# DefaultRui/VLN-VER

Measured on AMD Instinct MI355X. Metric: viewpoints/sec (multi-view->voxel fwd+bwd), vocc.py config, higher is better.
Workload: dtype bf16

## Files before the change

vln-ver_amd/csrc/ver_wgrad.hip:

```cpp
#include <cstdlib>
#include "ver_common.h"

namespace {
typedef __bf16 bf16x8 __attribute__((ext_vector_type(8)));
typedef float f32x16 __attribute__((ext_vector_type(16)));
typedef short s16x4 __attribute__((ext_vector_type(4)));
typedef short s16x8 __attribute__((ext_vector_type(8)));
typedef __attribute__((address_space(3))) s16x4 lds_s16x4;
typedef __attribute__((address_space(3))) void lds_void;

constexpr int kTile = 256;
constexpr int kSlabRows = 16;
constexpr int kSlabBytes = 2 * kSlabRows * kTile * 2;
constexpr int kRing = 8;
constexpr int kLdsBytes = kRing * kSlabBytes;

typedef int i32x2 __attribute__((ext_vector_type(2)));
typedef int i32x4 __attribute__((ext_vector_type(4)));

template <int OFF>
__device__ __forceinline__ i32x2 tr_read(int addr) {
    i32x2 v;
    asm volatile("ds_read_b64_tr_b16 %0, %1 offset:%2" : "=v"(v) : "v"(addr), "n"(OFF) : "memory");
    return v;
}
__device__ __forceinline__ bf16x8 frag(i32x2 lo, i32x2 hi) {
    return __builtin_bit_cast(bf16x8, (i32x4)__builtin_shufflevector(lo, hi, 0, 1, 2, 3));
}

struct WgradArgs {
    const __bf16* A;
    const __bf16* G;
    float* ws;
    long lda, ldg, M, Mc;
    int S, Ka, N, tiles_n, T;
    void* out;
    long ldo;
    int out_bf16;
    const __bf16* lattice;
    long lattice_bytes;
    const __bf16* cst;
    long cst_bytes;
    int B, H, W, C, P, CW, ncst, nseg;
    int seg_start[65];
    signed char kind[64], dz[64], dy[64], dx[64];
};

constexpr int kOutsideW = (int)0x80000000;
template <int L>
__device__ __forceinline__ int wcell_off(const WgradArgs& t, int b, int zl, int y, int x, int dz) {
    if ((unsigned)y >= (unsigned)t.H || (unsigned)x >= (unsigned)t.W) return kOutsideW;
    const int j = dz >> 1;
    int v;
    if (L == 0)
        v = ((b * 4 + zl + dz) * t.H + y) * t.W + x;
    else if (L == 2)
        v = ((((b * 2 + zl) * t.H + y) * t.W + x) << 1) + j;
    else
        v = (((((((y & 1) << 1 | (x & 1)) * t.B + b) * 2 + zl) * (t.H >> 1) + (y >> 1)) * (t.W >> 1) + (x >> 1)) << 1) + j;
    return v * t.C * 2;
}

struct WTapLane {
    int taddr;
    int boff;
    int bstep;
    int pend;
    int tend;
    int rows_left;
    int vo;
};

template <int L>
__device__ __forceinline__ int wtap_table_entry(const WgradArgs& t, int seg, int pos) {
    if (seg < 0) return kOutsideW;
    if (t.kind[seg]) return (pos * t.ncst + t.dz[seg]) * t.CW * 2;
    const int hw = t.H * t.W;
    const int zl = pos / hw, rem = pos - zl * hw;
    const int y = rem / t.W, x = rem - y * t.W;
    return wcell_off<L>(t, 0, zl, y + t.dy[seg], x + t.dx[seg], t.dz[seg]);
}

__device__ __forceinline__ int lds_read_b32(int addr) {
    int v;
    asm volatile("ds_read_b32 %0, %1" : "=v"(v) : "v"(addr) : "memory");
    return v;
}

__device__ __forceinline__ void wtap_step(const WgradArgs& t, WTapLane& tl, int tfetched) {
    tl.boff += tl.pend;
    tl.rows_left -= kSlabRows;
    tl.vo = tl.rows_left > 0 ? (int)((unsigned)tfetched + (unsigned)tl.boff) : kOutsideW;
    tl.taddr += 4 * kSlabRows;
    tl.pend = 0;
    if (tl.taddr >= tl.tend) tl.taddr -= 4 * t.P, tl.pend = tl.bstep;
}

struct WgradLane {
    int offA0, offA1, offB0, offB1;
    int voA, voG;
    int stepA, stepG;
    int dmaoff;
};

template <int SLOT>
__device__ __forceinline__ void read_slab(const WgradLane& c, i32x2 (&al)[4], i32x2 (&ah)[4], i32x2 (&bl)[2], i32x2 (&bh)[2]) {
    constexpr int SB = (SLOT & 3) * kSlabBytes;
    constexpr int UP = SLOT >= 4 ? 65536 : 0;
    const int a0 = c.offA0 + UP, a1 = c.offA1 + UP, b0 = c.offB0 + UP, b1 = c.offB1 + UP;
    al[0] = tr_read<SB>(a0);
    ah[0] = tr_read<SB + 512>(a0);
    bl[0] = tr_read<SB>(b0);
    bh[0] = tr_read<SB + 512>(b0);
    al[1] = tr_read<SB>(a1);
    ah[1] = tr_read<SB + 512>(a1);
    bl[1] = tr_read<SB>(b1);
    bh[1] = tr_read<SB + 512>(b1);
    al[2] = tr_read<SB + 1024>(a0);
    ah[2] = tr_read<SB + 1536>(a0);
    al[3] = tr_read<SB + 1024>(a1);
    ah[3] = tr_read<SB + 1536>(a1);
}

template <int PS, int KP, int PF, int IMPL>
__device__ __forceinline__ void phase(char* lds, f32x16 (&acc)[4][2], const WgradLane& c, __amdgpu_buffer_rsrc_t ra,
                                      __amdgpu_buffer_rsrc_t rg, unsigned& soA, unsigned& soG, const WgradArgs& t, WTapLane& tl) {
    i32x2 al[KP][4], ah[KP][4], bl[KP][2], bh[KP][2];
    int tnext = 0;
    read_slab<PS * KP>(c, al[0], ah[0], bl[0], bh[0]);
    if constexpr (KP == 2) read_slab<PS * KP + 1>(c, al[KP - 1], ah[KP - 1], bl[KP - 1], bh[KP - 1]);
#pragma unroll
    for (int u = 0; u < KP; ++u) {
        const int ds = (PS * KP + u + PF) % kRing;
        if constexpr (IMPL < 0) {
            __builtin_amdgcn_raw_ptr_buffer_load_lds(ra, (lds_void*)(lds + ds * kSlabBytes + c.dmaoff), 16, c.voA, (int)soA, 0, 0);
        } else {
            static_assert(IMPL < 0 || KP == 1, "implicit A: one slab per phase");
            __builtin_amdgcn_raw_ptr_buffer_load_lds(ra, (lds_void*)(lds + ds * kSlabBytes + c.dmaoff), 16, tl.vo, 0, 0, 0);
            tnext = lds_read_b32(tl.taddr);
        }
        __builtin_amdgcn_raw_ptr_buffer_load_lds(rg, (lds_void*)(lds + ds * kSlabBytes + kSlabBytes / 2 + c.dmaoff), 16, c.voG, (int)soG, 0, 0);
        soA += (unsigned)c.stepA;
        soG += (unsigned)c.stepG;
    }
    asm volatile("s_waitcnt vmcnt(%0)" ::"n"(2 * (PF - KP)) : "memory");
    __builtin_amdgcn_s_barrier();
    asm volatile("s_waitcnt lgkmcnt(0)"
                 : "+v"(al[0][0]), "+v"(ah[0][0]), "+v"(al[0][1]), "+v"(ah[0][1]), "+v"(al[0][2]), "+v"(ah[0][2]), "+v"(al[0][3]),
                   "+v"(ah[0][3]), "+v"(bl[0][0]), "+v"(bh[0][0]), "+v"(bl[0][1]), "+v"(bh[0][1]), "+v"(tnext)
                 :
                 : "memory");

    if constexpr (KP == 2)
        asm volatile(""
                     : "+v"(al[KP - 1][0]), "+v"(ah[KP - 1][0]), "+v"(al[KP - 1][1]), "+v"(ah[KP - 1][1]), "+v"(al[KP - 1][2]),
                       "+v"(ah[KP - 1][2]), "+v"(al[KP - 1][3]), "+v"(ah[KP - 1][3]), "+v"(bl[KP - 1][0]), "+v"(bh[KP - 1][0]),
                       "+v"(bl[KP - 1][1]), "+v"(bh[KP - 1][1])
                     :
                     : "memory");
    bf16x8 a[KP][4], b[KP][2];
#pragma unroll
    for (int u = 0; u < KP; ++u) {
#pragma unroll
        for (int i = 0; i < 4; ++i) a[u][i] = frag(al[u][i], ah[u][i]);
        b[u][0] = frag(bl[u][0], bh[u][0]);
        b[u][1] = frag(bl[u][1], bh[u][1]);
    }
    __builtin_amdgcn_sched_barrier(0);
    __builtin_amdgcn_s_setprio(1);
#pragma unroll
    for (int u = 0; u < KP; ++u)
#pragma unroll
        for (int it = 0; it < 4; ++it)
#pragma unroll
            for (int jt = 0; jt < 2; ++jt)
                acc[it][jt] = __builtin_amdgcn_mfma_f32_32x32x16_bf16(a[u][it], b[u][jt], acc[it][jt], 0, 0, 0);
    __builtin_amdgcn_s_setprio(0);
    __builtin_amdgcn_sched_barrier(0);
    if constexpr (IMPL >= 0) {
        wtap_step(t, tl, tnext);
        __builtin_amdgcn_sched_barrier(0);
    }
    __builtin_amdgcn_s_barrier();
}

template <int PS, int KP, int PF, int IMPL>
__device__ __forceinline__ void phases_from(int left, char* lds, f32x16 (&acc)[4][2], const WgradLane& c,
                                            __amdgpu_buffer_rsrc_t ra, __amdgpu_buffer_rsrc_t rg, unsigned& soA, unsigned& soG,
                                            const WgradArgs& t, WTapLane& tl) {
    if constexpr (PS < kRing / KP) {
        if (left > PS * KP) {
            phase<PS, KP, PF, IMPL>(lds, acc, c, ra, rg, soA, soG, t, tl);
            phases_from<PS + 1, KP, PF, IMPL>(left, lds, acc, c, ra, rg, soA, soG, t, tl);
        }
    }
}

template <int KP, int PF, int IMPL>
__device__ __forceinline__ void wgrad_body(const WgradArgs& p) {
    static_assert(PF >= KP && PF + (KP == 1 ? 2 : 4) <= kRing, "prefetch distance against the ring (WAR on the slot)");
    extern __shared__ __attribute__((aligned(1024))) char lds[];
    const int tid = threadIdx.x, lane = tid & 63;
    const int wave = __builtin_amdgcn_readfirstlane(tid >> 6);
    const int wr = wave >> 2, wc = wave & 3;
    int chunk, tile;
    {
        const int b = blockIdx.x;
        if ((p.S & 7) == 0) {
            const int xcd = b & 7, idx = b >> 3;
            chunk = xcd + 8 * (idx / p.T);
            tile = idx % p.T;
        } else {
            chunk = b / p.T;
            tile = b % p.T;
        }
    }
    const int mt = tile / p.tiles_n, nt = tile - mt * p.tiles_n;
    const long row0 = (long)chunk * p.Mc;
    const long rows = max(0L, min(p.Mc, p.M - row0));
    const int nslab = (int)((rows + kSlabRows * KP - 1) / (kSlabRows * KP)) * KP;

    const __bf16* ab = IMPL < 0 ? p.A + row0 * p.lda + (long)mt * kTile : nullptr;
    const __bf16* gb = p.G + row0 * p.ldg + (long)nt * kTile;
    const long abytes = ((p.M - row0 - 1) * p.lda + p.Ka - (long)mt * kTile) * 2;
    const long gbytes = ((p.M - row0 - 1) * p.ldg + p.N - (long)nt * kTile) * 2;
    const __amdgpu_buffer_rsrc_t rg = __builtin_amdgcn_make_buffer_rsrc((void*)gb, 0, (int)max(0L, min(gbytes, 0xFFFFFFFFL)), 0x00020000);
    WgradLane c;
    const int prow = lane >> 3, pch = (lane & 7) ^ (((prow >> 1) & 1) << 2);
    WTapLane tl = {};
    bool a_cst = false;
    if constexpr (IMPL >= 0) {
        int* tables = reinterpret_cast<int*>(lds + kLdsBytes);
        auto seg_of = [&](int col0) {
            int seg = -1;
            for (int i = 0; i < p.nseg; ++i)
                if (col0 >= p.seg_start[i] && col0 < p.seg_start[i + 1]) seg = i;
            return seg;
        };
        for (int q = 0; q < 4; ++q) {
            const int seg = seg_of(mt * kTile + 64 * q);
            for (int i = tid; i < p.P; i += 512) tables[q * p.P + i] = wtap_table_entry<IMPL>(p, seg, i);
        }
        __syncthreads();
        const int col0 = mt * kTile + 64 * (wave & 3);
        const int seg = seg_of(col0);
        a_cst = seg >= 0 && p.kind[seg];
        const long r = row0 + 8 * (wave >> 2) + prow;
        const int b0 = (int)(r / p.P), pos0 = (int)(r - (long)b0 * p.P);
        tl.bstep = a_cst ? 0 : (IMPL == 3 ? p.H * p.W : 4 * p.H * p.W) * p.C * 2;
        tl.boff = b0 * tl.bstep + (seg < 0 ? 0 : (col0 - p.seg_start[seg]) * 2) + pch * 16;
        const int lbase = (int)(uintptr_t)(__attribute__((address_space(3))) char*)(lds + kLdsBytes) + (wave & 3) * p.P * 4;
        tl.tend = lbase + 4 * p.P;
        tl.taddr = lbase + 4 * pos0;
        tl.pend = 0;
        tl.rows_left = (int)min(min(p.M, row0 + p.Mc) - r, 0x7FFFFFF0L) + kSlabRows;
        int t0 = lds_read_b32(tl.taddr);
        asm volatile("s_waitcnt lgkmcnt(0)" : "+v"(t0)::"memory");
        wtap_step(p, tl, t0);
    }
    const __amdgpu_buffer_rsrc_t ra =
        IMPL < 0 ? __builtin_amdgcn_make_buffer_rsrc((void*)ab, 0, (int)max(0L, min(abytes, 0xFFFFFFFFL)), 0x00020000)
                 : __builtin_amdgcn_make_buffer_rsrc((void*)(a_cst ? p.cst : p.lattice), 0,
                                                     (int)max(0L, min(a_cst ? p.cst_bytes : p.lattice_bytes, 0x7FFFFFFFL)), 0x00020000);
    c.voA = (int)(((8 * (wave >> 2) + prow) * p.lda + 64 * (wave & 3)) * 2) + pch * 16;
    c.voG = (int)(((8 * (wave >> 2) + prow) * p.ldg + 64 * (wave & 3)) * 2) + pch * 16;
    c.stepA = (int)(kSlabRows * p.lda * 2);
    c.stepG = (int)(kSlabRows * p.ldg * 2);
    c.dmaoff = wave * 1024;
    unsigned soA = 0, soG = 0;

    {
        const int q = lane >> 4, cl = lane & 15;
        const int lowch = (2 * (q & 1) + ((cl & 3) >> 1)) ^ (((cl >> 3) & 1) << 2);
        const int lbase = (int)(uintptr_t)(__attribute__((address_space(3))) char*)lds;
        const int rowoff = lbase + ((q >> 1) * 32 + (cl >> 2)) * 128 + lowch * 16 + (cl & 1) * 8;
        c.offA0 = rowoff + 2 * wr * 1024;
        c.offA1 = c.offA0 ^ 64;
        c.offB0 = rowoff + wc * 1024 + kSlabBytes / 2;
        c.offB1 = c.offB0 ^ 64;
    }

    f32x16 acc[4][2];
#pragma unroll
    for (int it = 0; it < 4; ++it)
#pragma unroll
        for (int jt = 0; jt < 2; ++jt)
#pragma unroll
            for (int r = 0; r < 16; ++r) acc[it][jt][r] = 0.0f;

#pragma unroll
    for (int s = 0; s < PF; ++s) {
        if constexpr (IMPL < 0) {
            __builtin_amdgcn_raw_ptr_buffer_load_lds(ra, (lds_void*)(lds + s * kSlabBytes + c.dmaoff), 16, c.voA, (int)soA, 0, 0);
        } else {
            __builtin_amdgcn_raw_ptr_buffer_load_lds(ra, (lds_void*)(lds + s * kSlabBytes + c.dmaoff), 16, tl.vo, 0, 0, 0);
            int tn = lds_read_b32(tl.taddr);
            asm volatile("s_waitcnt lgkmcnt(0)" : "+v"(tn)::"memory");
            wtap_step(p, tl, tn);
        }
        __builtin_amdgcn_raw_ptr_buffer_load_lds(rg, (lds_void*)(lds + s * kSlabBytes + kSlabBytes / 2 + c.dmaoff), 16, c.voG, (int)soG, 0, 0);
        soA += (unsigned)c.stepA;
        soG += (unsigned)c.stepG;
    }
    asm volatile("s_waitcnt vmcnt(%0)" ::"n"(2 * (PF - KP)) : "memory");
    __builtin_amdgcn_s_barrier();
    if (wr == 1) __builtin_amdgcn_s_barrier();

    int s = 0;
    for (; s + kRing <= nslab; s += kRing) phases_from<0, KP, PF, IMPL>(kRing, lds, acc, c, ra, rg, soA, soG, p, tl);
    phases_from<0, KP, PF, IMPL>(nslab - s, lds, acc, c, ra, rg, soA, soG, p, tl);
    if (wr == 0) __builtin_amdgcn_s_barrier();
    asm volatile("s_waitcnt vmcnt(0)" ::: "memory");

    const int i0 = mt * kTile + 128 * wr + 4 * (lane >> 5), j0 = nt * kTile + 64 * wc + (lane & 31);
    if (p.S == 1 && p.out) {
#pragma unroll
        for (int it = 0; it < 4; ++it)
#pragma unroll
            for (int jt = 0; jt < 2; ++jt) {
                const int j = j0 + 32 * jt;
#pragma unroll
                for (int r = 0; r < 16; ++r) {
                    const int i = i0 + 32 * it + (r & 3) + 8 * (r >> 2);
                    if (i < p.Ka && j < p.N) {
                        if (p.out_bf16)
                            reinterpret_cast<__bf16*>(p.out)[(long)i * p.ldo + j] = (__bf16)acc[it][jt][r];
                        else
                            reinterpret_cast<float*>(p.out)[(long)i * p.ldo + j] = acc[it][jt][r];
                    }
                }
            }
        return;
    }
    float* out = p.ws + (long)chunk * p.Ka * p.N;
#pragma unroll
    for (int it = 0; it < 4; ++it)
#pragma unroll
        for (int jt = 0; jt < 2; ++jt) {
            const int j = j0 + 32 * jt;
#pragma unroll
            for (int r = 0; r < 16; ++r) {
                const int i = i0 + 32 * it + (r & 3) + 8 * (r >> 2);
                if (i < p.Ka && j < p.N) out[(long)i * p.N + j] = acc[it][jt][r];
            }
        }
}

template <int KP, int PF>
__global__ __launch_bounds__(512) void k_wgrad_tn(WgradArgs p) {
    wgrad_body<KP, PF, -1>(p);
}

template <int L, int PF>
__global__ __launch_bounds__(512) void k_wgrad_tn_seg(WgradArgs p) {
    wgrad_body<1, PF, L>(p);
}

template <typename OT>
__global__ __launch_bounds__(256) void k_wgrad_reduce(const float* __restrict__ ws, OT* __restrict__ out, long ldo, int S,
                                                      int Ka, int N) {
    const long n4 = (long)Ka * N / 4;
    const long stride = (long)Ka * N;
    for (long e = blockIdx.x * 256L + threadIdx.x; e < n4; e += (long)gridDim.x * 256) {
        float4 acc = *reinterpret_cast<const float4*>(ws + 4 * e);
        for (int s = 1; s < S; ++s) {
            const float4 v = *reinterpret_cast<const float4*>(ws + s * stride + 4 * e);
            acc.x += v.x;
            acc.y += v.y;
            acc.z += v.z;
            acc.w += v.w;
        }
        const long i = (4 * e) / N, j = (4 * e) - i * N;
        OT* o = out + i * ldo + j;
        if constexpr (sizeof(OT) == 4) {
            *reinterpret_cast<float4*>(o) = acc;
        } else {
            typedef __bf16 bf16x4 __attribute__((ext_vector_type(4)));
            bf16x4 v;
            v.x = (__bf16)acc.x;
            v.y = (__bf16)acc.y;
            v.z = (__bf16)acc.z;
            v.w = (__bf16)acc.w;
            *reinterpret_cast<bf16x4*>(o) = v;
        }
    }
}

long max_chunk_rows(long ld) {
    if (ld <= 0) return 45000;
    const long rows = (0xFFFFFFFFL / (ld * 2)) - 16 * kRing - 2 * kSlabRows - 1;
    return rows < 45000 ? (rows > 2 * kSlabRows ? rows : 2 * kSlabRows) : 45000;
}

int pick_splits(long M, int Ka, int N, long ld = 0) {
    const long cap = max_chunk_rows(ld);
    const long tiles = (long)((Ka + kTile - 1) / kTile) * ((N + kTile - 1) / kTile);
    static const int cand[] = {1, 2, 3, 4, 6, 8, 12, 16, 24, 32, 48, 64};
    int best = 0;
    double best_us = 0.0;
    for (int s : cand) {
        if ((M + s - 1) / s > cap) continue;
        if (s > 1 && M / s < 256) break;
        if (M > 32768 && s % 8) continue;
        const long rounds = (tiles * s + 255) / 256;
        const double slabs = (double)((M + s - 1) / s + 15) / 16.0;
        double us = (double)rounds * (slabs * 0.37 + 8.0) + (s == 1 ? 0.25 : (double)s) * (double)Ka * (double)N * 8.0 / 3.0e6;
        if (s % 8 == 0) us *= 0.97;
        if (!best || us < best_us) {
            best = s;
            best_us = us;
        }
    }
    if (!best) {
        best = 64;
        while (best < 65536 && (M + best - 1) / best > cap) best *= 2;
    }
    return best;
}

template <int KP, int PF>
void launch_tn(const WgradArgs& p, int blocks, hipStream_t st, hipError_t& e) {
    auto kern = k_wgrad_tn<KP, PF>;
    e = hipFuncSetAttribute((const void*)kern, hipFuncAttributeMaxDynamicSharedMemorySize, kLdsBytes);
    if (e == hipSuccess) hipLaunchKernelGGL(kern, dim3((unsigned)blocks), dim3(512), kLdsBytes, st, p);
}
template <int L, int PF>
void launch_tn_segments_pf(const WgradArgs& p, int blocks, hipStream_t st, hipError_t& e) {
    const int ldsb = kLdsBytes + 4 * p.P * 4;
    e = hipFuncSetAttribute((const void*)k_wgrad_tn_seg<L, PF>, hipFuncAttributeMaxDynamicSharedMemorySize, ldsb);
    if (e == hipSuccess) hipLaunchKernelGGL((k_wgrad_tn_seg<L, PF>), dim3((unsigned)blocks), dim3(512), ldsb, st, p);
}

template <int L>
void launch_tn_segments(const WgradArgs& p, int blocks, hipStream_t st, hipError_t& e) {
    static const int pf = [] {
        const char* v = getenv("VER_WGRAD_SEG_PF");
        return v ? atoi(v) : 3;
    }();
    if (pf == 4) launch_tn_segments_pf<L, 4>(p, blocks, st, e);
    else if (pf == 5) launch_tn_segments_pf<L, 5>(p, blocks, st, e);
    else if (pf == 6) launch_tn_segments_pf<L, 6>(p, blocks, st, e);
    else launch_tn_segments_pf<L, 3>(p, blocks, st, e);
}
}

extern "C" int ver_wgrad_tn_splits(long M, int Ka, int N) {
    if (M <= 0 || Ka <= 0 || N <= 0) return 1;
    return pick_splits(M, Ka, N);
}

extern "C" int ver_wgrad_tn_splits_ld(long M, int Ka, int N, long ld) {
    if (M <= 0 || Ka <= 0 || N <= 0) return 1;
    return pick_splits(M, Ka, N, ld);
}

extern "C" long ver_wgrad_tn_workspace(long M, int Ka, int N, int splits) {
    if (Ka <= 0 || N <= 0) return 0;
    if (splits <= 0) splits = ver_wgrad_tn_splits(M, Ka, N);
    return (long)splits * Ka * N * (long)sizeof(float);
}

extern "C" int ver_wgrad_tn(const void* a, long lda, const void* g, long ldg, long M, int Ka, int N, void* out, long ldo,
                            int out_dtype, int splits, int flags, void* workspace, long workspace_bytes, void* stream) {
    hipStream_t st = (hipStream_t)stream;
    VER_REQUIRE(M >= 0 && Ka > 0 && N > 0, VER_EINVAL, "ver_wgrad_tn: bad sizes M=%ld Ka=%d N=%d", M, Ka, N);
    VER_REQUIRE(out && workspace && ((a && g) || M == 0), VER_EINVAL, "ver_wgrad_tn: null pointer argument");
    VER_REQUIRE(out_dtype == VER_F32 || out_dtype == VER_BF16, VER_EINVAL, "ver_wgrad_tn: out_dtype %d", out_dtype);
    VER_REQUIRE(lda >= Ka && ldg >= N && ldo >= N, VER_EINVAL, "ver_wgrad_tn: row pitch smaller than the row");
    VER_REQUIRE(lda % 8 == 0 && ldg % 8 == 0 && ((uintptr_t)a & 15) == 0 && ((uintptr_t)g & 15) == 0, VER_EUNSUPPORTED,
                "ver_wgrad_tn: operands must be 16-byte aligned with row pitches that are multiples of 8 elements");
    VER_REQUIRE(N % 4 == 0 && ldo % 4 == 0 && ((uintptr_t)out & 15) == 0, VER_EUNSUPPORTED,
                "ver_wgrad_tn: N and the output pitch must be multiples of 4");
    const int S = splits > 0 ? splits : pick_splits(M, Ka, N, lda > ldg ? lda : ldg);
    VER_REQUIRE(S <= 65536, VER_EINVAL, "ver_wgrad_tn: %d row chunks", S);
    const long Mc = ((M + S - 1) / S + 2 * kSlabRows - 1) / (2 * kSlabRows) * (2 * kSlabRows);
    VER_REQUIRE((Mc + 16 * kRing) * (lda > ldg ? lda : ldg) * 2 < 0xFFFFFFFFL, VER_EUNSUPPORTED,
                "ver_wgrad_tn: a row chunk exceeds the 4-GiB range of a buffer offset (more splits)");
    VER_REQUIRE(workspace_bytes >= (long)S * Ka * N * (long)sizeof(float), VER_EINVAL, "ver_wgrad_tn: workspace of %ld bytes, %ld needed",
                workspace_bytes, (long)S * Ka * N * (long)sizeof(float));
    WgradArgs p = {};
    p.A = (const __bf16*)a;
    p.G = (const __bf16*)g;
    p.ws = (float*)workspace;
    p.lda = lda;
    p.ldg = ldg;
    p.M = M;
    p.Mc = Mc;
    p.S = S;
    p.Ka = Ka;
    p.N = N;
    p.tiles_n = (N + kTile - 1) / kTile;
    p.T = ((Ka + kTile - 1) / kTile) * p.tiles_n;
    const bool direct = S == 1 && M > 0;
    p.out = direct ? out : nullptr;
    p.ldo = ldo;
    p.out_bf16 = out_dtype == VER_BF16;
    hipError_t e = hipSuccess;
    if (M > 0) {
        switch (flags & 15) {
            case 4: launch_tn<1, 4>(p, p.T * S, st, e); break;
            case 5: launch_tn<1, 5>(p, p.T * S, st, e); break;
            case 6: launch_tn<1, 6>(p, p.T * S, st, e); break;
            case 8 + 2: launch_tn<2, 2>(p, p.T * S, st, e); break;
            case 8 + 4: launch_tn<2, 4>(p, p.T * S, st, e); break;
            default: launch_tn<1, 3>(p, p.T * S, st, e); break;
        }
        if (e != hipSuccess) return ver_fail(VER_ELAUNCH, "ver_wgrad_tn: LDS attribute: %s", hipGetErrorString(e));
    } else if (int zrc = ver_zero_async(workspace, (size_t)S * Ka * N * sizeof(float), st)) {
        return zrc;
    }
    if (direct) return ver_check_launch("ver_wgrad_tn");
    const long n4 = (long)Ka * N / 4;
    long grid = (n4 + 255) / 256;
    if (grid > 8192) grid = 8192;
    if (out_dtype == VER_F32)
        hipLaunchKernelGGL(k_wgrad_reduce<float>, dim3((unsigned)grid), dim3(256), 0, st, (const float*)workspace, (float*)out, ldo, S, Ka, N);
    else
        hipLaunchKernelGGL(k_wgrad_reduce<__bf16>, dim3((unsigned)grid), dim3(256), 0, st, (const float*)workspace, (__bf16*)out, ldo, S, Ka, N);
    return ver_check_launch("ver_wgrad_tn");
}

extern "C" int ver_wgrad_tn_segments(const void* lattice, int layout, int B, int H, int W, int C, const int* taps, int nseg,
                                     const void* cst, int ncst, int cw, const void* g, long ldg, int N, void* out, long ldo,
                                     int out_dtype, int splits, void* workspace, long workspace_bytes, void* stream) {
    hipStream_t st = (hipStream_t)stream;
    VER_REQUIRE(B >= 0 && H > 0 && W > 0 && C > 0 && N > 0 && nseg > 0, VER_EINVAL, "ver_wgrad_tn_segments: bad sizes");
    VER_REQUIRE(layout == 0 || layout == 2 || layout == 3, VER_EINVAL, "ver_wgrad_tn_segments: layout %d (0 plain, 2 z-split, 3 planar z-split)", layout);
    VER_REQUIRE(layout != 3 || (H % 2 == 0 && W % 2 == 0), VER_EINVAL, "ver_wgrad_tn_segments: planar needs even H, W");
    VER_REQUIRE(out && workspace && ((lattice && g && taps) || B == 0), VER_EINVAL, "ver_wgrad_tn_segments: null pointer argument");
    VER_REQUIRE(out_dtype == VER_F32 || out_dtype == VER_BF16, VER_EINVAL, "ver_wgrad_tn_segments: out_dtype %d", out_dtype);
    VER_REQUIRE(nseg <= 64, VER_EUNSUPPORTED, "ver_wgrad_tn_segments: %d segments (at most 64)", nseg);
    VER_REQUIRE(C % 64 == 0 && (cst == nullptr || (ncst > 0 && ncst <= 64 && cw > 0 && cw % 64 == 0 && ((uintptr_t)cst & 15) == 0)),
                VER_EUNSUPPORTED, "ver_wgrad_tn_segments: segment widths (C = %d, pattern blocks of %d) must be multiples of 64", C, cw);
    const long M = (long)B * 2 * H * W, lbytes = (long)B * 4 * H * W * C * 2;
    const int P = 2 * H * W;
    VER_REQUIRE(P >= kSlabRows && P <= 2048 && lbytes < 0x7FFFFFFFL, VER_EUNSUPPORTED,
                "ver_wgrad_tn_segments: %d rows per viewpoint / a source lattice of %ld bytes (16 <= rows <= 2048: four offset tables "
                "next to the 128-KB ring in LDS; below 2 GiB)", P, lbytes);
    VER_REQUIRE(ldg >= N && ldo >= N && ldg % 8 == 0 && ((uintptr_t)g & 15) == 0 && ((uintptr_t)lattice & 15) == 0, VER_EUNSUPPORTED,
                "ver_wgrad_tn_segments: g must be 16-byte aligned with a row pitch that is a multiple of 8 elements");
    VER_REQUIRE(N % 4 == 0 && ldo % 4 == 0 && ((uintptr_t)out & 15) == 0, VER_EUNSUPPORTED,
                "ver_wgrad_tn_segments: N and the output pitch must be multiples of 4");
    WgradArgs p = {};
    long Ka = 0;
    for (int i = 0; i < nseg; ++i) {
        const int dz = taps[3 * i], dy = taps[3 * i + 1], dx = taps[3 * i + 2];
        p.seg_start[i] = (int)Ka;
        if (dz < 0) {
            VER_REQUIRE(cst && -1 - dz < ncst, VER_EINVAL, "ver_wgrad_tn_segments: segment %d names pattern block %d of %d", i, -1 - dz, cst ? ncst : 0);
            p.kind[i] = 1, p.dz[i] = (signed char)(-1 - dz);
            Ka += cw;
        } else {
            VER_REQUIRE((dz == 0 || dz == 2) && dy >= -64 && dy <= 64 && dx >= -64 && dx <= 64, VER_EINVAL,
                        "ver_wgrad_tn_segments: tap %d = (%d, %d, %d): dz must be 0 or 2", i, dz, dy, dx);
            p.kind[i] = 0, p.dz[i] = (signed char)dz, p.dy[i] = (signed char)dy, p.dx[i] = (signed char)dx;
            Ka += C;
        }
    }
    p.seg_start[nseg] = (int)Ka;
    VER_REQUIRE(Ka < 0x7FFFFFFFL, VER_EUNSUPPORTED, "ver_wgrad_tn_segments: %ld columns", Ka);
    const int S = splits > 0 ? splits : pick_splits(M, (int)Ka, N, ldg);
    VER_REQUIRE(S <= 65536, VER_EINVAL, "ver_wgrad_tn_segments: %d row chunks", S);
    const long Mc = ((M + S - 1) / S + 2 * kSlabRows - 1) / (2 * kSlabRows) * (2 * kSlabRows);
    VER_REQUIRE((Mc + 16 * kRing) * ldg * 2 < 0xFFFFFFFFL, VER_EUNSUPPORTED,
                "ver_wgrad_tn_segments: a row chunk exceeds the 4-GiB range of a buffer offset (more splits)");
    VER_REQUIRE(workspace_bytes >= (long)S * Ka * N * (long)sizeof(float), VER_EINVAL, "ver_wgrad_tn_segments: workspace of %ld bytes, %ld needed",
                workspace_bytes, (long)S * Ka * N * (long)sizeof(float));
    p.A = nullptr;
    p.G = (const __bf16*)g;
    p.ws = (float*)workspace;
    p.lda = 0;
    p.ldg = ldg;
    p.M = M;
    p.Mc = Mc;
    p.S = S;
    p.Ka = (int)Ka;
    p.N = N;
    p.tiles_n = (N + kTile - 1) / kTile;
    p.T = (int)((Ka + kTile - 1) / kTile) * p.tiles_n;
    const bool direct = S == 1 && M > 0;
    p.out = direct ? out : nullptr;
    p.ldo = ldo;
    p.out_bf16 = out_dtype == VER_BF16;
    p.lattice = (const __bf16*)lattice;
    p.lattice_bytes = lbytes;
    p.cst = (const __bf16*)cst;
    p.cst_bytes = cst ? (long)P * ncst * cw * 2 : 0;
    p.B = B, p.H = H, p.W = W, p.C = C, p.P = P, p.CW = cw, p.ncst = ncst, p.nseg = nseg;
    hipError_t e = hipSuccess;
    if (M > 0) {
        if (layout == 0) launch_tn_segments<0>(p, p.T * S, st, e);
        else if (layout == 2) launch_tn_segments<2>(p, p.T * S, st, e);
        else launch_tn_segments<3>(p, p.T * S, st, e);
        if (e != hipSuccess) return ver_fail(VER_ELAUNCH, "ver_wgrad_tn_segments: LDS attribute: %s", hipGetErrorString(e));
    } else if (int zrc = ver_zero_async(workspace, (size_t)S * Ka * N * sizeof(float), st)) {
        return zrc;
    }
    if (direct) return ver_check_launch("ver_wgrad_tn_segments");
    const long n4 = Ka * N / 4;
    long grid = (n4 + 255) / 256;
    if (grid > 8192) grid = 8192;
    if (out_dtype == VER_F32)
        hipLaunchKernelGGL(k_wgrad_reduce<float>, dim3((unsigned)grid), dim3(256), 0, st, (const float*)workspace, (float*)out, ldo, S, (int)Ka, N);
    else
        hipLaunchKernelGGL(k_wgrad_reduce<__bf16>, dim3((unsigned)grid), dim3(256), 0, st, (const float*)workspace, (__bf16*)out, ldo, S, (int)Ka, N);
    return ver_check_launch("ver_wgrad_tn_segments");
}

extern "C" int ver_wgrad_tn_segments_splits(int B, int H, int W, long Ka, int N, long ldg) {
    const long M = (long)B * 2 * H * W;
    if (M <= 0 || Ka <= 0 || N <= 0) return 1;
    return pick_splits(M, (int)Ka, N, ldg);
}
```

Before: 679.7.

## Switch weight-gradient kernel from 32x32x16 to 16x16x32 MFMA with slab-pair k-steps

Re-tiles the weight-gradient GEMM (dense and lattice-segment paths) to use 16x16x32 bf16 MFMA instead of 32x32x16. Each phase now consumes a pair of slabs as one k-step, with new LDS fragment offsets and a modified swizzle, and a two-slot tap walker keeps the implicit-A gather addresses for both slabs. The prefetch distance becomes 4, and the env/flag-selected prefetch variants are removed. The aim is better MFMA throughput or latency for this shape, at the cost of more accumulator registers per wave, a new LDS bank pattern, and a riskier index calculation.

```diff
diff --git a/scratch/gemm_mfma_shape_ab.py b/scratch/gemm_mfma_shape_ab.py
--- /dev/null
+++ b/scratch/gemm_mfma_shape_ab.py
@@ -0,0 +1,102 @@
+import argparse
+import ctypes
+import json
+import os
+import shutil
+import statistics
+import sys
+import tempfile
+
+import torch
+
+M, K, N = 345600, 14304, 1536
+c_long, c_int, c_void = ctypes.c_long, ctypes.c_int, ctypes.c_void_p
+
+
+def load(path):
+    L = ctypes.CDLL(path)
+    L.ver_gemm_nn.argtypes = [c_void, c_long, c_void, c_long, c_void, c_void, c_long, c_long, c_int, c_int, c_int, c_void]
+    L.ver_wgrad_tn.argtypes = [c_void, c_long, c_void, c_long, c_long, c_int, c_int, c_void, c_long, c_int, c_int, c_int, c_void,
+                               c_long, c_void]
+    L.ver_wgrad_tn_splits_ld.argtypes = [c_long, c_int, c_int, c_long]
+    L.ver_wgrad_tn_workspace.argtypes = [c_long, c_int, c_int, c_int]
+    L.ver_wgrad_tn_workspace.restype = c_long
+    return L
+
+
+def timed(f, n=6):
+    for _ in range(2):
+        f()
+    torch.cuda.synchronize()
+    a, b = torch.cuda.Event(enable_timing=True), torch.cuda.Event(enable_timing=True)
+    a.record()
+    for _ in range(n):
+        f()
+    b.record()
+    torch.cuda.synchronize()
+    return a.elapsed_time(b) / n
+
+
+def main():
+    ap = argparse.ArgumentParser()
+    ap.add_argument('parent')
+    ap.add_argument('new')
+    ap.add_argument('--reps', type=int, default=5)
+    ap.add_argument('--out', default=None)
+    ap.add_argument('--families', default='gemm_nn,wgrad_tn')
+    args = ap.parse_args()
+    tmp = tempfile.mkdtemp()
+    copy = shutil.copy(args.parent, os.path.join(tmp, 'libver_hip_parent_copy.so'))
+    arms = [('parent', load(args.parent)), ('new', load(args.new)), ('parent_copy', load(copy))]
+    dev = 'cuda'
+    st = torch.cuda.current_stream().cuda_stream
+    out = open(args.out, 'a') if args.out else None
+
+    def emit(rec):
+        line = json.dumps(rec)
+        print(line, flush=True)
+        if out:
+            out.write(line + '\n')
+            out.flush()
+
+    def check(rc, what):
+        if rc != 0:
+            sys.exit('%s returned %d' % (what, rc))
+
+    makes = (('N(0,1)', lambda *s: torch.randn(*s, device=dev).bfloat16()),
+             ('constant 0.5', lambda *s: torch.full(s, 0.5, device=dev, dtype=torch.bfloat16)),
+             ('zeros', lambda *s: torch.zeros(*s, device=dev, dtype=torch.bfloat16)))
+    fl = 2.0 * M * K * N
+    for dist, make in makes:
+        a, g, w = make(M, K), make(M, N), make(K, N)
+        c = torch.empty(M, N, dtype=torch.bfloat16, device=dev)
+        dw = torch.empty(K, N, dtype=torch.bfloat16, device=dev)
+        for fam in args.families.split(','):
+            samples = {name: [] for name, _ in arms}
+            for _ in range(args.reps):
+                for name, L in arms:
+                    if fam == 'gemm_nn':
+                        f = lambda: check(L.ver_gemm_nn(a.data_ptr(), K, w.data_ptr(), N, None, c.data_ptr(), N, M, K, N, 0, st), fam)
+                    else:
+                        s = L.ver_wgrad_tn_splits_ld(M, K, N, K)
+                        nb = L.ver_wgrad_tn_workspace(M, K, N, s)
+                        ws = torch.empty(nb // 4, dtype=torch.float32, device=dev)
+                        f = lambda: check(L.ver_wgrad_tn(a.data_ptr(), K, g.data_ptr(), N, M, K, N, dw.data_ptr(), N, 1, s, 0,
+                                                         ws.data_ptr(), nb, st), fam)
+                    samples[name].append(timed(f))
+            med = {k: statistics.median(v) for k, v in samples.items()}
+            for name, _ in arms:
+                emit(dict(kind='microbench', family=fam, operands=dist, arm=name, M=M, K=K, N=N, ms=[round(x, 4) for x in samples[name]],
+                          ms_median=round(med[name], 4), tflops=round(fl / med[name] / 1e9, 1)))
+            spread = abs(med['parent'] - med['parent_copy'])
+            gain = med['parent'] - med['new']
+            emit(dict(kind='verdict', family=fam, operands=dist, parent_ms=round(med['parent'], 4), new_ms=round(med['new'], 4),
+                      parent_aa_spread_ms=round(spread, 4), gain_ms=round(gain, 4), speedup=round(med['parent'] / med['new'], 4),
+                      clears_twice_the_spread=bool(gain > 2 * spread)))
+        del a, g, w, c, dw
+        torch.cuda.empty_cache()
+    shutil.rmtree(tmp, ignore_errors=True)
+
+
+if __name__ == '__main__':
+    main()
diff --git a/scratch/lattice_mfma_shape_ab.py b/scratch/lattice_mfma_shape_ab.py
--- /dev/null
+++ b/scratch/lattice_mfma_shape_ab.py
@@ -0,0 +1,94 @@
+import argparse
+import importlib
+import json
+import os
+import shutil
+import statistics
+import sys
+import tempfile
+
+import torch
+
+ROOT = os.path.dirname(os.path.dirname(os.path.abspath(__file__)))
+sys.path.insert(0, ROOT)
+hip = importlib.import_module('vln-ver_amd.hipops')
+ups = importlib.import_module('vln-ver_amd.dense_heads.upsample')
+
+
+def load(path):
+    hip._lib, hip.LIB_PATH = None, os.path.abspath(path)
+    return hip.lib()
+
+
+def timed(f, n=5):
+    f()
+    torch.cuda.synchronize()
+    a, b = torch.cuda.Event(enable_timing=True), torch.cuda.Event(enable_timing=True)
+    a.record()
+    for _ in range(n):
+        f()
+    b.record()
+    torch.cuda.synchronize()
+    return a.elapsed_time(b) / n
+
+
+def main():
+    ap = argparse.ArgumentParser()
+    ap.add_argument('arms', nargs='+', help='name=path; the first is the parent')
+    ap.add_argument('--reps', type=int, default=5)
+    ap.add_argument('--out', default=None)
+    args = ap.parse_args()
+    arms = [a.split('=', 1) for a in args.arms]
+    tmp = tempfile.mkdtemp()
+    arms.append(['parent_copy', shutil.copy(arms[0][1], os.path.join(tmp, 'libver_hip_parent_copy.so'))])
+    handles = [(name, load(path)) for name, path in arms]
+    out = open(args.out, 'a') if args.out else None
+
+    def emit(rec):
+        line = json.dumps(rec)
+        print(line, flush=True)
+        if out:
+            out.write(line + '\n')
+            out.flush()
+
+    B, DEV, C, N, layout, hc = 192, 'cuda', 768, 1536, 3, 30
+    plan = ups._layer_plan_z4(C, torch.device(DEV))[0]
+    m = B * 2 * hc * hc
+    e = torch.randn(4, B, 2, hc // 2, hc // 2, 2, C, device=DEV).bfloat16()
+    table, _ = ups._const_rows_z4(C, hc, hc, torch.device(DEV), torch.bfloat16)
+    g = torch.randn(m, N, device=DEV).bfloat16()
+    cls = [(ups._class_segments_z4(c, C), plan[c][1] - plan[c][0]) for c in ups._CLASSES]
+    ws = [torch.randn(k, N, device=DEV).bfloat16() for _, k in cls]
+    dws = [torch.empty(k, N, dtype=torch.bfloat16, device=DEV) for _, k in cls]
+    y = torch.empty(m, N, dtype=torch.bfloat16, device=DEV)
+    flops = 2.0 * m * N * sum(k for _, k in cls)
+
+    def forward():
+        for (segs, _), w in zip(cls, ws):
+            hip.gemm_nn_taps(e, layout, (hc, hc), segs, w, const_rows=table, out=y)
+
+    def wgrad():
+        for (segs, _), dw in zip(cls, dws):
+            hip.wgrad_tn_segments(e, layout, (hc, hc), segs, g, out=dw, const_rows=table)
+
+    for fam, f in (('gemm_nn_segments', forward), ('wgrad_tn_segments', wgrad)):
+        samples = {name: [] for name, _ in handles}
+        for _ in range(args.reps):
+            for name, h in handles:
+                hip._lib = h
+                samples[name].append(timed(f))
+        med = {k: statistics.median(v) for k, v in samples.items()}
+        spread = abs(med[arms[0][0]] - med['parent_copy'])
+        for name, _ in handles:
+            emit(dict(kind='microbench', family=fam, operands='N(0,1)', arm=name, M=m, K=sum(k for _, k in cls), N=N,
+                      ms=[round(x, 4) for x in samples[name]], ms_median=round(med[name], 4), tflops=round(flops / med[name] / 1e9, 1)))
+        for name, _ in handles[1:-1]:
+            gain = med[arms[0][0]] - med[name]
+            emit(dict(kind='verdict', family=fam, operands='N(0,1)', arm=name, parent_ms=round(med[arms[0][0]], 4), new_ms=round(med[name], 4),
+                      parent_aa_spread_ms=round(spread, 4), gain_ms=round(gain, 4), speedup=round(med[arms[0][0]] / med[name], 4),
+                      clears_twice_the_spread=bool(gain > 2 * spread)))
+    shutil.rmtree(tmp, ignore_errors=True)
+
+
+if __name__ == '__main__':
+    main()
diff --git a/vln-ver_amd/csrc/ver_wgrad.hip b/vln-ver_amd/csrc/ver_wgrad.hip
--- a/vln-ver_amd/csrc/ver_wgrad.hip
+++ b/vln-ver_amd/csrc/ver_wgrad.hip
@@ -1,9 +1,9 @@
-#include <cstdlib>
 #include "ver_common.h"
 
 namespace {
 typedef __bf16 bf16x8 __attribute__((ext_vector_type(8)));
 typedef float f32x16 __attribute__((ext_vector_type(16)));
+typedef float f32x4 __attribute__((ext_vector_type(4)));
 typedef short s16x4 __attribute__((ext_vector_type(4)));
 typedef short s16x8 __attribute__((ext_vector_type(8)));
 typedef __attribute__((address_space(3))) s16x4 lds_s16x4;
@@ -17,6 +17,24 @@
 
 typedef int i32x2 __attribute__((ext_vector_type(2)));
 typedef int i32x4 __attribute__((ext_vector_type(4)));
+
+constexpr int kShape = 16;
+template <int SH>
+struct Shape {
+    typedef f32x16 acc_t;
+    static constexpr int NI = 4, NJ = 2, NR = 16, TW = 32;
+    static __device__ __forceinline__ int reg_row(int r) { return (r & 3) + 8 * (r >> 2); }
+    static __device__ __forceinline__ int lane_row(int lane) { return 4 * (lane >> 5); }
+    static __device__ __forceinline__ int swz(int row, int rowhalf) { return ((row >> 1) & 1) << 2; }
+};
+template <>
+struct Shape<16> {
+    typedef f32x4 acc_t;
+    static constexpr int NI = 8, NJ = 4, NR = 4, TW = 16;
+    static __device__ __forceinline__ int reg_row(int r) { return r; }
+    static __device__ __forceinline__ int lane_row(int lane) { return 4 * (lane >> 4); }
+    static __device__ __forceinline__ int swz(int row, int rowhalf) { return (((row >> 1) & 1) << 2) ^ (rowhalf << 1); }
+};
 
 template <int OFF>
 __device__ __forceinline__ i32x2 tr_read(int addr) {
@@ -69,6 +87,7 @@
     int tend;
     int rows_left;
     int vo;
+    int taddr1, pend1, vo1;
 };
 
 template <int L>
@@ -96,8 +115,23 @@
     if (tl.taddr >= tl.tend) tl.taddr -= 4 * t.P, tl.pend = tl.bstep;
 }
 
+__device__ __forceinline__ void wtap_step2(const WgradArgs& t, WTapLane& tl, int tfetched0, int tfetched1) {
+    tl.boff += tl.pend;
+    tl.rows_left -= kSlabRows;
+    tl.vo = tl.rows_left > 0 ? (int)((unsigned)tfetched0 + (unsigned)tl.boff) : kOutsideW;
+    tl.boff += tl.pend1;
+    tl.rows_left -= kSlabRows;
+    tl.vo1 = tl.rows_left > 0 ? (int)((unsigned)tfetched1 + (unsigned)tl.boff) : kOutsideW;
+    tl.taddr = tl.taddr1 + 4 * kSlabRows;
+    tl.pend = 0;
+    if (tl.taddr >= tl.tend) tl.taddr -= 4 * t.P, tl.pend = tl.bstep;
+    tl.taddr1 = tl.taddr + 4 * kSlabRows;
+    tl.pend1 = 0;
+    if (tl.taddr1 >= tl.tend) tl.taddr1 -= 4 * t.P, tl.pend1 = tl.bstep;
+}
+
 struct WgradLane {
-    int offA0, offA1, offB0, offB1;
+    int offA[4], offB[4];
     int voA, voG;
     int stepA, stepG;
     int dmaoff;
@@ -107,7 +141,7 @@
 __device__ __forceinline__ void read_slab(const WgradLane& c, i32x2 (&al)[4], i32x2 (&ah)[4], i32x2 (&bl)[2], i32x2 (&bh)[2]) {
     constexpr int SB = (SLOT & 3) * kSlabBytes;
     constexpr int UP = SLOT >= 4 ? 65536 : 0;
-    const int a0 = c.offA0 + UP, a1 = c.offA1 + UP, b0 = c.offB0 + UP, b1 = c.offB1 + UP;
+    const int a0 = c.offA[0] + UP, a1 = c.offA[1] + UP, b0 = c.offB[0] + UP, b1 = c.offB[1] + UP;
     al[0] = tr_read<SB>(a0);
     ah[0] = tr_read<SB + 512>(a0);
     bl[0] = tr_read<SB>(b0);
@@ -123,6 +157,67 @@
 }
 
 template <int PS, int KP, int PF, int IMPL>
+__device__ __forceinline__ void phase(char* lds, f32x4 (&acc)[8][4], const WgradLane& c, __amdgpu_buffer_rsrc_t ra,
+                                      __amdgpu_buffer_rsrc_t rg, unsigned& soA, unsigned& soG, const WgradArgs& t, WTapLane& tl) {
+    static_assert(KP == 2, "16x16x32: a k-step is a slab pair");
+    constexpr int SB = ((2 * PS) & 3) * kSlabBytes;
+    constexpr int UP = 2 * PS >= 4 ? 65536 : 0;
+    i32x2 al[8], ah[8], bl[4], bh[4];
+    int tn0 = 0, tn1 = 0;
+#pragma unroll
+    for (int q = 0; q < 4; ++q) {
+        const int a = c.offA[q] + UP, b = c.offB[q] + UP;
+        al[q] = tr_read<SB>(a);
+        ah[q] = tr_read<SB + 512>(a);
+        bl[q] = tr_read<SB>(b);
+        bh[q] = tr_read<SB + 512>(b);
+        al[4 + q] = tr_read<SB + 1024>(a);
+        ah[4 + q] = tr_read<SB + 1536>(a);
+    }
+#pragma unroll
+    for (int u = 0; u < 2; ++u) {
+        const int ds = (2 * PS + u + PF) % kRing;
+        if constexpr (IMPL < 0) {
+            __builtin_amdgcn_raw_ptr_buffer_load_lds(ra, (lds_void*)(lds + ds * kSlabBytes + c.dmaoff), 16, c.voA, (int)soA, 0, 0);
+        } else {
+            __builtin_amdgcn_raw_ptr_buffer_load_lds(ra, (lds_void*)(lds + ds * kSlabBytes + c.dmaoff), 16, u ? tl.vo1 : tl.vo, 0, 0, 0);
+            if (u) tn1 = lds_read_b32(tl.taddr1);
+            else tn0 = lds_read_b32(tl.taddr);
+        }
+        __builtin_amdgcn_raw_ptr_buffer_load_lds(rg, (lds_void*)(lds + ds * kSlabBytes + kSlabBytes / 2 + c.dmaoff), 16, c.voG, (int)soG, 0, 0);
+        soA += (unsigned)c.stepA;
+        soG += (unsigned)c.stepG;
+    }
+    asm volatile("s_waitcnt vmcnt(%0)" ::"n"(2 * (PF - KP)) : "memory");
+    __builtin_amdgcn_s_barrier();
+    asm volatile("s_waitcnt lgkmcnt(0)"
+                 : "+v"(al[0]), "+v"(ah[0]), "+v"(al[1]), "+v"(ah[1]), "+v"(al[2]), "+v"(ah[2]), "+v"(al[3]), "+v"(ah[3]), "+v"(al[4]),
+                   "+v"(ah[4]), "+v"(al[5]), "+v"(ah[5]), "+v"(al[6]), "+v"(ah[6]), "+v"(al[7]), "+v"(ah[7]), "+v"(bl[0]), "+v"(bh[0]),
+                   "+v"(bl[1]), "+v"(bh[1]), "+v"(bl[2]), "+v"(bh[2]), "+v"(bl[3]), "+v"(bh[3]), "+v"(tn0), "+v"(tn1)
+                 :
+                 : "memory");
+    bf16x8 a[8], b[4];
+#pragma unroll
+    for (int i = 0; i < 8; ++i) a[i] = frag(al[i], ah[i]);
+#pragma unroll
+    for (int j = 0; j < 4; ++j) b[j] = frag(bl[j], bh[j]);
+    __builtin_amdgcn_sched_barrier(0);
+    __builtin_amdgcn_s_setprio(1);
+#pragma unroll
+    for (int it = 0; it < 8; ++it)
+#pragma unroll
+        for (int jt = 0; jt < 4; ++jt)
+            acc[it][jt] = __builtin_amdgcn_mfma_f32_16x16x32_bf16(a[it], b[jt], acc[it][jt], 0, 0, 0);
+    __builtin_amdgcn_s_setprio(0);
+    __builtin_amdgcn_sched_barrier(0);
+    if constexpr (IMPL >= 0) {
+        wtap_step2(t, tl, tn0, tn1);
+        __builtin_amdgcn_sched_barrier(0);
+    }
+    __builtin_amdgcn_s_barrier();
+}
+
+template <int PS, int KP, int PF, int IMPL>
 __device__ __forceinline__ void phase(char* lds, f32x16 (&acc)[4][2], const WgradLane& c, __amdgpu_buffer_rsrc_t ra,
                                       __amdgpu_buffer_rsrc_t rg, unsigned& soA, unsigned& soG, const WgradArgs& t, WTapLane& tl) {
     i32x2 al[KP][4], ah[KP][4], bl[KP][2], bh[KP][2];
@@ -184,8 +279,8 @@
     __builtin_amdgcn_s_barrier();
 }
 
-template <int PS, int KP, int PF, int IMPL>
-__device__ __forceinline__ void phases_from(int left, char* lds, f32x16 (&acc)[4][2], const WgradLane& c,
+template <int PS, int KP, int PF, int IMPL, typename ACC>
+__device__ __forceinline__ void phases_from(int left, char* lds, ACC& acc, const WgradLane& c,
                                             __amdgpu_buffer_rsrc_t ra, __amdgpu_buffer_rsrc_t rg, unsigned& soA, unsigned& soG,
                                             const WgradArgs& t, WTapLane& tl) {
     if constexpr (PS < kRing / KP) {
@@ -196,9 +291,11 @@
     }
 }
 
-template <int KP, int PF, int IMPL>
+template <int SH, int KP, int PF, int IMPL>
 __device__ __forceinline__ void wgrad_body(const WgradArgs& p) {
+    typedef Shape<SH> sh;
     static_assert(PF >= KP && PF + (KP == 1 ? 2 : 4) <= kRing, "prefetch distance against the ring (WAR on the slot)");
+    static_assert(SH == 32 || KP == 2, "16x16x32: a k-step is a slab pair");
     extern __shared__ __attribute__((aligned(1024))) char lds[];
     const int tid = threadIdx.x, lane = tid & 63;
     const int wave = __builtin_amdgcn_readfirstlane(tid >> 6);
@@ -226,7 +323,7 @@
     const long gbytes = ((p.M - row0 - 1) * p.ldg + p.N - (long)nt * kTile) * 2;
     const __amdgpu_buffer_rsrc_t rg = __builtin_amdgcn_make_buffer_rsrc((void*)gb, 0, (int)max(0L, min(gbytes, 0xFFFFFFFFL)), 0x00020000);
     WgradLane c;
-    const int prow = lane >> 3, pch = (lane & 7) ^ (((prow >> 1) & 1) << 2);
+    const int prow = lane >> 3, pch = (lane & 7) ^ sh::swz(prow, wave >> 2);
     WTapLane tl = {};
     bool a_cst = false;
     if constexpr (IMPL >= 0) {
@@ -269,24 +366,35 @@
     c.dmaoff = wave * 1024;
     unsigned soA = 0, soG = 0;
 
-    {
+    if constexpr (SH == 32) {
         const int q = lane >> 4, cl = lane & 15;
-        const int lowch = (2 * (q & 1) + ((cl & 3) >> 1)) ^ (((cl >> 3) & 1) << 2);
+        const int lowch = (2 * (q & 1) + ((cl & 3) >> 1)) ^ sh::swz(cl >> 2, q >> 1);
         const int lbase = (int)(uintptr_t)(__attribute__((address_space(3))) char*)lds;
         const int rowoff = lbase + ((q >> 1) * 32 + (cl >> 2)) * 128 + lowch * 16 + (cl & 1) * 8;
-        c.offA0 = rowoff + 2 * wr * 1024;
-        c.offA1 = c.offA0 ^ 64;
-        c.offB0 = rowoff + wc * 1024 + kSlabBytes / 2;
-        c.offB1 = c.offB0 ^ 64;
-    }
-
-    f32x16 acc[4][2];
-#pragma unroll
-    for (int it = 0; it < 4; ++it)
-#pragma unroll
-        for (int jt = 0; jt < 2; ++jt)
-#pragma unroll
-            for (int r = 0; r < 16; ++r) acc[it][jt][r] = 0.0f;
+        c.offA[0] = rowoff + 2 * wr * 1024;
+        c.offA[1] = c.offA[0] ^ 64;
+        c.offB[0] = rowoff + wc * 1024 + kSlabBytes / 2;
+        c.offB[1] = c.offB[0] ^ 64;
+        c.offA[2] = c.offA[3] = c.offB[2] = c.offB[3] = 0;
+    } else {
+        const int g = lane >> 4, cl = lane & 15;
+        const int lbase = (int)(uintptr_t)(__attribute__((address_space(3))) char*)lds;
+#pragma unroll
+        for (int q = 0; q < 4; ++q) {
+            const int ch = (2 * q + ((cl & 3) >> 1)) ^ sh::swz(cl >> 2, g & 1);
+            const int rowoff = lbase + (g >> 1) * kSlabBytes + (g & 1) * 4096 + (cl >> 2) * 128 + ch * 16 + (cl & 1) * 8;
+            c.offA[q] = rowoff + 2 * wr * 1024;
+            c.offB[q] = rowoff + wc * 1024 + kSlabBytes / 2;
+        }
+    }
+
+    typename sh::acc_t acc[sh::NI][sh::NJ];
+#pragma unroll
+    for (int it = 0; it < sh::NI; ++it)
+#pragma unroll
+        for (int jt = 0; jt < sh::NJ; ++jt)
+#pragma unroll
+            for (int r = 0; r < sh::NR; ++r) acc[it][jt][r] = 0.0f;
 
 #pragma unroll
     for (int s = 0; s < PF; ++s) {
@@ -302,6 +410,17 @@
         soA += (unsigned)c.stepA;
         soG += (unsigned)c.stepG;
     }
+    if constexpr (IMPL >= 0 && KP == 2) {
+        const int vo0 = tl.vo;
+        int tn = lds_read_b32(tl.taddr);
+        asm volatile("s_waitcnt lgkmcnt(0)" : "+v"(tn)::"memory");
+        wtap_step(p, tl, tn);
+        tl.vo1 = tl.vo;
+        tl.vo = vo0;
+        tl.taddr1 = tl.taddr + 4 * kSlabRows;
+        tl.pend1 = 0;
+        if (tl.taddr1 >= tl.tend) tl.taddr1 -= 4 * p.P, tl.pend1 = tl.bstep;
+    }
     asm volatile("s_waitcnt vmcnt(%0)" ::"n"(2 * (PF - KP)) : "memory");
     __builtin_amdgcn_s_barrier();
     if (wr == 1) __builtin_amdgcn_s_barrier();
@@ -312,16 +431,16 @@
     if (wr == 0) __builtin_amdgcn_s_barrier();
     asm volatile("s_waitcnt vmcnt(0)" ::: "memory");
 
-    const int i0 = mt * kTile + 128 * wr + 4 * (lane >> 5), j0 = nt * kTile + 64 * wc + (lane & 31);
+    const int i0 = mt * kTile + 128 * wr + sh::lane_row(lane), j0 = nt * kTile + 64 * wc + (lane & (sh::TW - 1));
     if (p.S == 1 && p.out) {
 #pragma unroll
-        for (int it = 0; it < 4; ++it)
-#pragma unroll
-            for (int jt = 0; jt < 2; ++jt) {
-                const int j = j0 + 32 * jt;
-#pragma unroll
-                for (int r = 0; r < 16; ++r) {
-                    const int i = i0 + 32 * it + (r & 3) + 8 * (r >> 2);
+        for (int it = 0; it < sh::NI; ++it)
+#pragma unroll
+            for (int jt = 0; jt < sh::NJ; ++jt) {
+                const int j = j0 + sh::TW * jt;
+#pragma unroll
+                for (int r = 0; r < sh::NR; ++r) {
+                    const int i = i0 + sh::TW * it + sh::reg_row(r);
                     if (i < p.Ka && j < p.N) {
                         if (p.out_bf16)
                             reinterpret_cast<__bf16*>(p.out)[(long)i * p.ldo + j] = (__bf16)acc[it][jt][r];
@@ -334,26 +453,29 @@
     }
     float* out = p.ws + (long)chunk * p.Ka * p.N;
 #pragma unroll
-    for (int it = 0; it < 4; ++it)
-#pragma unroll
-        for (int jt = 0; jt < 2; ++jt) {
-            const int j = j0 + 32 * jt;
-#pragma unroll
-            for (int r = 0; r < 16; ++r) {
-                const int i = i0 + 32 * it + (r & 3) + 8 * (r >> 2);
+    for (int it = 0; it < sh::NI; ++it)
+#pragma unroll
+        for (int jt = 0; jt < sh::NJ; ++jt) {
+            const int j = j0 + sh::TW * jt;
+#pragma unroll
+            for (int r = 0; r < sh::NR; ++r) {
+                const int i = i0 + sh::TW * it + sh::reg_row(r);
                 if (i < p.Ka && j < p.N) out[(long)i * p.N + j] = acc[it][jt][r];
             }
         }
 }
 
-template <int KP, int PF>
+constexpr int kKP = kShape == 16 ? 2 : 1;
+constexpr int kPF = kShape == 16 ? 4 : 3;
+
+template <int SH>
 __global__ __launch_bounds__(512) void k_wgrad_tn(WgradArgs p) {
-    wgrad_body<KP, PF, -1>(p);
-}
-
-template <int L, int PF>
+    wgrad_body<SH, kKP, kPF, -1>(p);
+}
+
+template <int L, int SH>
 __global__ __launch_bounds__(512) void k_wgrad_tn_seg(WgradArgs p) {
-    wgrad_body<1, PF, L>(p);
+    wgrad_body<SH, kKP, kPF, L>(p);
 }
 
 template <typename OT>
@@ -418,29 +540,17 @@
     return best;
 }
 
-template <int KP, int PF>
 void launch_tn(const WgradArgs& p, int blocks, hipStream_t st, hipError_t& e) {
-    auto kern = k_wgrad_tn<KP, PF>;
+    auto kern = k_wgrad_tn<kShape>;
     e = hipFuncSetAttribute((const void*)kern, hipFuncAttributeMaxDynamicSharedMemorySize, kLdsBytes);
     if (e == hipSuccess) hipLaunchKernelGGL(kern, dim3((unsigned)blocks), dim3(512), kLdsBytes, st, p);
 }
-template <int L, int PF>
-void launch_tn_segments_pf(const WgradArgs& p, int blocks, hipStream_t st, hipError_t& e) {
-    const int ldsb = kLdsBytes + 4 * p.P * 4;
-    e = hipFuncSetAttribute((const void*)k_wgrad_tn_seg<L, PF>, hipFuncAttributeMaxDynamicSharedMemorySize, ldsb);
-    if (e == hipSuccess) hipLaunchKernelGGL((k_wgrad_tn_seg<L, PF>), dim3((unsigned)blocks), dim3(512), ldsb, st, p);
-}
 
 template <int L>
 void launch_tn_segments(const WgradArgs& p, int blocks, hipStream_t st, hipError_t& e) {
-    static const int pf = [] {
-        const char* v = getenv("VER_WGRAD_SEG_PF");
-        return v ? atoi(v) : 3;
-    }();
-    if (pf == 4) launch_tn_segments_pf<L, 4>(p, blocks, st, e);
-    else if (pf == 5) launch_tn_segments_pf<L, 5>(p, blocks, st, e);
-    else if (pf == 6) launch_tn_segments_pf<L, 6>(p, blocks, st, e);
-    else launch_tn_segments_pf<L, 3>(p, blocks, st, e);
+    const int ldsb = kLdsBytes + 4 * p.P * 4;
+    e = hipFuncSetAttribute((const void*)k_wgrad_tn_seg<L, kShape>, hipFuncAttributeMaxDynamicSharedMemorySize, ldsb);
+    if (e == hipSuccess) hipLaunchKernelGGL((k_wgrad_tn_seg<L, kShape>), dim3((unsigned)blocks), dim3(512), ldsb, st, p);
 }
 }
 
@@ -466,6 +576,7 @@
     VER_REQUIRE(M >= 0 && Ka > 0 && N > 0, VER_EINVAL, "ver_wgrad_tn: bad sizes M=%ld Ka=%d N=%d", M, Ka, N);
     VER_REQUIRE(out && workspace && ((a && g) || M == 0), VER_EINVAL, "ver_wgrad_tn: null pointer argument");
     VER_REQUIRE(out_dtype == VER_F32 || out_dtype == VER_BF16, VER_EINVAL, "ver_wgrad_tn: out_dtype %d", out_dtype);
+    VER_REQUIRE(flags == 0, VER_EINVAL, "ver_wgrad_tn: unknown flags 0x%x", flags);
     VER_REQUIRE(lda >= Ka && ldg >= N && ldo >= N, VER_EINVAL, "ver_wgrad_tn: row pitch smaller than the row");
     VER_REQUIRE(lda % 8 == 0 && ldg % 8 == 0 && ((uintptr_t)a & 15) == 0 && ((uintptr_t)g & 15) == 0, VER_EUNSUPPORTED,
                 "ver_wgrad_tn: operands must be 16-byte aligned with row pitches that are multiples of 8 elements");
@@ -497,14 +608,7 @@
     p.out_bf16 = out_dtype == VER_BF16;
     hipError_t e = hipSuccess;
     if (M > 0) {
-        switch (flags & 15) {
-            case 4: launch_tn<1, 4>(p, p.T * S, st, e); break;
-            case 5: launch_tn<1, 5>(p, p.T * S, st, e); break;
-            case 6: launch_tn<1, 6>(p, p.T * S, st, e); break;
-            case 8 + 2: launch_tn<2, 2>(p, p.T * S, st, e); break;
-            case 8 + 4: launch_tn<2, 4>(p, p.T * S, st, e); break;
-            default: launch_tn<1, 3>(p, p.T * S, st, e); break;
-        }
+        launch_tn(p, p.T * S, st, e);
         if (e != hipSuccess) return ver_fail(VER_ELAUNCH, "ver_wgrad_tn: LDS attribute: %s", hipGetErrorString(e));
     } else if (int zrc = ver_zero_async(workspace, (size_t)S * Ka * N * sizeof(float), st)) {
         return zrc;
```

After: 688.6, median of 6. +1.3%, better.
